# batra-mlp-lab/visdial

Hardware: AMD Instinct MI355X
Metric: QA-rounds/sec training mn-att-ques-im-hist+disc (batch 20x10x100) (higher is better)
Workload: dtype f32 operands and results; the option recurrence multiplies the EXACT 3-way bf16 split of both operands (9 bf16 MFMA products per fp32 product, f32 accumulate: fp32-grade, errors at the f32 MFMA's own level) -- its two step kernels and its weight-gradient contraction; f32 MFMA (v_mfma_f32_32x32x2_f32

## Files before the change

### visdial_amd/csrc/lstm.hip

```cpp
#include "gemm_core.h"
#include "split_core.h"

extern "C" int vd_gemm_tn_acc(const float* A, int64_t lda, const float* B, int64_t ldb, float* C, int64_t ldc, int M,
                              int N, int K, int flags, void* stream);

#define VD_LSTM_CELL(E, PI, PF, PO, PG, CP)   \
  gi.E = km * vd_sigmoid(PI);                 \
  gf.E = km * vd_sigmoid(PF);                 \
  go.E = km * vd_sigmoid(PO);                 \
  gg.E = km * vd_tanh(PG);                    \
  c.E = gf.E * (CP) + gi.E * gg.E;            \
  h.E = go.E * vd_tanh(c.E);
#define VD_XYZW(M) M(x) M(y) M(z) M(w)
#define VD_ADD4(a, b) a.x += b.x; a.y += b.y; a.z += b.z; a.w += b.w;

template <bool C16 = false>
struct EpiLstmFwdT {
  const float* xproj;
  long xld;
  const int* tok_gather;
  const int* tok_mask;
  const float* c_prev;
  float* gates;
  float* c_out;
// ... 322 lines not shown
  __device__ __forceinline__ long kstep() const { return 1; }
};

#define VD_LSTM_GRAD(E, G, CT, CP, DCV, LTR)                                                                   \
  {                                                                                                            \
    float gi_ = G[0].E, gf_ = G[1].E, go_ = G[2].E;                                                            \
    float pi_ = 0.f, pf_ = 0.f, po_ = 0.f;                              \
    if constexpr (!(LTR)) pi_ = gi_ * (1.f - gi_), pf_ = gf_ * (1.f - gf_), po_ = go_ * (1.f - go_);           \
    if constexpr (C16) {                \
      pi_ = gi_ < 0.f ? (1.f + gi_) * -gi_ : pi_;  gi_ = gi_ < 0.f ? 1.f + gi_ : gi_;                          \
      pf_ = gf_ < 0.f ? (1.f + gf_) * -gf_ : pf_;  gf_ = gf_ < 0.f ? 1.f + gf_ : gf_;                          \
      po_ = go_ < 0.f ? (1.f + go_) * -go_ : po_;  go_ = go_ < 0.f ? 1.f + go_ : go_;                          \
    }                                                                                                          \
    const float tc = vd_tanh(CT.E);                                                                            \
    const float d = DCV.E + dh.E * go_ * (1.f - tc * tc);                                                      \
    ai.E = LTR ? d * G[3].E * gi_ * (1.f - gi_) : d * G[3].E * pi_;                                            \
    af.E = LTR ? d * CP.E * gf_ * (1.f - gf_) : d * CP.E * pf_;                                                \
    ao.E = LTR ? dh.E * tc * go_ * (1.f - go_) : dh.E * tc * po_;                                              \
    ag.E = d * gi_ * (1.f - G[3].E * G[3].E);                                                                  \
    dn.E = d * gf_;                                                                                            \
  }

template <int NT, int BATCH = (NT == 1 ? 2 : 1), bool TWO = true, bool C16 = false>
struct EpiLstmBwd {
  const float* dh_a;
  const float* dh_b;
  float* gates;
  const float* c_t;
  const float* c_prev;
  float* dc;
  int dc_first;
  int H;
  vd_bf16_bits* da16 = nullptr;
  static constexpr bool HAS_DIST = NT == 1 && !C16;
  struct DOps {
    float4 g[4], ct, cp, dcv, dha, dhb;
  };
  __device__ __forceinline__ bool dist_ok() const { return true; }
  __device__ __forceinline__ void dist_load(DOps& q, int row0, int col0, int lane, int grp, int M) const {
    const int j = col0 + (lane & 7) * 4;
    const int row = row0 + grp * 8 + (lane >> 3);
    const int rc = row < M ? row : M - 1;
    const long o = (long)rc * H + j;
    const float* gr = gates + (long)rc * 4 * H + j;
    const float4 z = make_float4(0.f, 0.f, 0.f, 0.f);
    q.g[0] = *reinterpret_cast<const float4*>(gr);
    q.g[1] = *reinterpret_cast<const float4*>(gr + H);
    q.g[2] = *reinterpret_cast<const float4*>(gr + 2 * H);
    q.g[3] = *reinterpret_cast<const float4*>(gr + 3 * H);
    q.ct = *reinterpret_cast<const float4*>(c_t + o);
    q.cp = c_prev ? *reinterpret_cast<const float4*>(c_prev + o) : z;
    q.dcv = dc_first ? z : *reinterpret_cast<const float4*>(dc + o);
    q.dha = dh_a ? *reinterpret_cast<const float4*>(dh_a + o) : z;
    q.dhb = dh_b ? *reinterpret_cast<const float4*>(dh_b + o) : z;
  }
  __device__ __forceinline__ void dist_store(const float4 (&a)[1], const DOps& q, int row0, int col0, int lane, int grp, int M) const {
    const int j = col0 + (lane & 7) * 4;
    const int row = row0 + grp * 8 + (lane >> 3);
    if (row >= M || j >= H) return;
    float4 dh = a[0], ai, af, ao, ag, dn;
    dh.x += q.dha.x + q.dhb.x; dh.y += q.dha.y + q.dhb.y; dh.z += q.dha.z + q.dhb.z; dh.w += q.dha.w + q.dhb.w;
#define VD_GRAD(E) VD_LSTM_GRAD(E, q.g, q.ct, q.cp, q.dcv, true)
    VD_XYZW(VD_GRAD)
#undef VD_GRAD
    float* gr = gates + (long)row * 4 * H + j;
    *reinterpret_cast<float4*>(gr) = ai;
// ... 10 lines not shown
    }
  }
  struct Slot {
    float4 g[4], ct, cp, dcv, dhx;
    vd_u32x2 g16[4];
  };
  struct Rsrc {
    __amdgpu_buffer_rsrc_t g, ct, cp, dc, dh1, dh2, g16;
  };
  __device__ __forceinline__ void load_slot_buf(Slot& L, const Rsrc& R, unsigned o4, unsigned og4, unsigned uH4) const {
    if constexpr (C16) {
      L.g16[0] = __builtin_amdgcn_raw_buffer_load_b64(R.g, og4 >> 1, 0, 0);
      L.g16[1] = __builtin_amdgcn_raw_buffer_load_b64(R.g, og4 >> 1, uH4 >> 1, 0);
      L.g16[2] = __builtin_amdgcn_raw_buffer_load_b64(R.g, og4 >> 1, uH4, 0);
      L.g16[3] = __builtin_amdgcn_raw_buffer_load_b64(R.g, og4 >> 1, 3 * (uH4 >> 1), 0);
    } else {
    L.g[0] = vd_buf_ld4(R.g, og4, 0);
    L.g[1] = vd_buf_ld4(R.g, og4, uH4);
    L.g[2] = vd_buf_ld4(R.g, og4, 2 * uH4);
    L.g[3] = vd_buf_ld4(R.g, og4, 3 * uH4);
    }
    L.ct = vd_buf_ld4(R.ct, o4, 0);
    const float4 z = make_float4(0.f, 0.f, 0.f, 0.f);
    L.cp = c_prev ? vd_buf_ld4(R.cp, o4, 0) : z;
    L.dcv = dc_first ? z : vd_buf_ld4(R.dc, o4, 0);
    L.dhx = (dh_a || dh_b) ? vd_buf_ld4(R.dh1, o4, 0) : z;
  }
  __device__ __forceinline__ void operator()(const f32x16 (&acc)[NT], int row0, int col0, int lane, int M,
                                             int N, float* scr) const {
    const int rl = lane >> 3, cl = (lane & 7) * 4;
    const bool two_dh = TWO && dh_a && dh_b;
    const Rsrc R{vd_rsrc(gates), vd_rsrc(c_t), vd_rsrc(c_prev), vd_rsrc(dc), vd_rsrc(dh_a ? dh_a : dh_b), vd_rsrc(dh_b), vd_rsrc(da16)};
    const unsigned uH4 = (unsigned)H * 4u;
#pragma unroll
    for (int jt = 0; jt < NT; ++jt) {
      float4 d4[4];
      tile_to_rows(acc[jt], scr, lane, d4);
      if (jt == 0) VD_T(3);
      const int j = col0 + jt * 32 + cl;
      const int jc = j < N ? j : N - 4;
#pragma unroll
      for (int pp = 0; pp < 4; pp += BATCH) {
        Slot L[BATCH];
        unsigned o4[BATCH], og4[BATCH];
#pragma unroll
        for (int q = 0; q < BATCH; ++q) {
          const int row = row0 + (pp + q) * 8 + rl;
          o4[q] = (unsigned)(row < M ? row : M - 1) * uH4 + (unsigned)jc * 4u;
          og4[q] = 4u * o4[q] - 12u * (unsigned)jc;
          load_slot_buf(L[q], R, o4[q], og4[q], uH4);
        }
        __builtin_amdgcn_sched_barrier(0);
#pragma unroll
        for (int q = 0; q < BATCH; ++q) {
          Slot& C = L[q];
          if constexpr (C16) {
#pragma unroll
            for (int gk = 0; gk < 4; ++gk) C.g[gk] = vd_bf16x4_unpack(C.g16[gk]);
          }
          float4 dh = d4[pp + q];
          VD_ADD4(dh, C.dhx)
          const int row = row0 + (pp + q) * 8 + rl;
          if constexpr (TWO) {
            if (two_dh) {
              const float4 t = vd_buf_ld4(R.dh2, o4[q], 0);
              VD_ADD4(dh, t)
            }
          }
          float4 ai, af, ao, ag, dn;
#define VD_GRAD(E) VD_LSTM_GRAD(E, C.g, C.ct, C.cp, C.dcv, false)
          VD_XYZW(VD_GRAD)
#undef VD_GRAD
          if (row < M && j < N) {
            if constexpr (C16) {
              vd_buf_st4_bf16(R.g, og4[q] >> 1, 0, ai);
              vd_buf_st4_bf16(R.g, og4[q] >> 1, uH4 >> 1, af);
              vd_buf_st4_bf16(R.g, og4[q] >> 1, uH4, ao);
              vd_buf_st4_bf16(R.g, og4[q] >> 1, 3 * (uH4 >> 1), ag);
            } else {
            vd_buf_st4(R.g, og4[q], 0, ai);
            vd_buf_st4(R.g, og4[q], uH4, af);
            vd_buf_st4(R.g, og4[q], 2 * uH4, ao);
            vd_buf_st4(R.g, og4[q], 3 * uH4, ag);
            }
            vd_buf_st4(R.dc, o4[q], 0, dn);
            if (!C16 && da16) {
              vd_buf_st4_bf16(R.g16, og4[q] >> 1, 0, ai);
              vd_buf_st4_bf16(R.g16, og4[q] >> 1, uH4 >> 1, af);
              vd_buf_st4_bf16(R.g16, og4[q] >> 1, uH4, ao);
              vd_buf_st4_bf16(R.g16, og4[q] >> 1, 3 * (uH4 >> 1), ag);
            }
          }
        }
      }
    }
  }
};

using CfgF9 = GemmCfg<4, 1, 4, 16, 0, 4, 41984>;
using CfgB1 = GemmCfg<4, 1, 4, 32, 0, 3>;
using CfgB11 = GemmCfg<4, 1, 2, 16, 0, 4, 41984>;
using CfgFbf16 = GemmCfg<4, 1, 4, 32, 0, 3, 0, 1>;
using CfgBbf16 = GemmCfg<4, 1, 2, 32, 0, 3, 0, 1>;
#ifndef VD_C16_LDS
#define VD_C16_LDS 41984
#endif
using CfgF9bf16 = GemmCfg<4, 1, 4, 16, 0, 4, VD_C16_LDS, 1>;
using CfgB11bf16 = GemmCfg<4, 1, 2, 16, 0, 4, VD_C16_LDS, 1>;
using CfgFwdSmallA = GemmCfg<1, 4, 4, 8, 0, 3>;
using CfgFwdSmallC = GemmCfg<1, 4, 4, 8, 0, 4>;
using CfgBwdSmallD = GemmCfg<1, 4, 1, 32, 2, 4>;
using CfgTickFwdBf16 = GemmCfg<1, 4, 4, 16, 0, 3, 0, 1>;
using CfgTickBwdBf16 = GemmCfg<1, 4, 1, 32, 0, 4, 0, 1>;

__global__ void __launch_bounds__(256) wh_gate_transpose_kernel(const float* __restrict__ Wh,
                                                                float* __restrict__ WhT, int H, int plain = 0) {
  __shared__ float tile[32][33];
  const int vt = blockIdx.x, kt = blockIdx.y;
  const int jb = vt >> 2, g = vt & 3;
  const int tx = threadIdx.x & 31, ty = threadIdx.x >> 5;
  const long src_col = plain ? (long)vt * 32 : (long)g * H + jb * 32;
#pragma unroll
  for (int i = 0; i < 4; ++i) {
    const int k = kt * 32 + ty + i * 8;
    tile[ty + i * 8][tx] = Wh[(long)k * 4 * H + src_col + tx];
  }
// ... 61 lines not shown
  const int N = P.N, H = P.H;
  if (h_prev) {
    if constexpr (Epi::STEP_BF16) {
      if (P.bf16 && t > 0)
        return launch_gemm_glds<CfgF9bf16, false>(N, 4 * H, H / 2, 1, reinterpret_cast<const float*>(P.h16 + (long)(t - 1) * N * H), (long)H / 2,
                                                  reinterpret_cast<const float*>(P.w.W16), (long)H / 2, epi, s);
      if (P.bf16) return launch_gemm<CfgFbf16>(N, 4 * H, H, 1, SrcRow{h_prev, H}, SrcRow{P.w.WhT, H}, epi, s);
    }
    if constexpr (Epi::STEP_SPLIT) {
      if (P.split) return launch_gemm_split(P.split, N, 4 * H, H, h_prev, (long)H, P.w.W3, (long)H, 4L * H * H, epi, s);
    }
    if (P.glds) return launch_gemm_glds<CfgF9, false>(N, 4 * H, H, 1, h_prev, (long)H, P.w.WhT, (long)H, epi, s);
  }
  auto generic = [&](auto a) {
    SrcKGate4 b{P.Wh, 4L * H, H};
    if (N >= VD_THROUGHPUT_ROWS) return launch_gemm<CfgF9>(N, 4 * H, h_prev ? H : 0, 1, a, b, epi, s);
    return launch_gemm<CfgFwdSmallA>(N, 4 * H, h_prev ? H : 0, 1, a, b, epi, s);
  };
  if constexpr (EpiARowsOf<Epi>::value) {
    if (h_prev) return generic(SrcRowTree{h_prev, H, epi.tok_mask, epi.parent});
  }
  return generic(SrcRow{h_prev, H});
}

struct LstmBwdPlan {
  int N, H;
  const float* Wh;
  int split;
  LstmWeights w;
  vd_bf16_bits* da16;
};
template <class E>
static E lstm_bwd_epi(const EpiLstmBwd<2>& e) {
  return E{e.dh_a, e.dh_b, e.gates, e.c_t, e.c_prev, e.dc, e.dc_first, e.H, e.da16};
}

static int lstm_step_bwd(const LstmBwdPlan& P, const float* da_next, const vd_bf16_bits* da16_next, const EpiLstmBwd<2>& e, hipStream_t s) {
  const int N = P.N, H = P.H, K = da_next ? 4 * H : 0;
  const bool one_dh = !(e.dh_a && e.dh_b);
  SrcRow a{da_next, 4L * H};
  SrcRow b{P.Wh, 4L * H};
  if (P.split && K > 0 && one_dh)
    return launch_gemm_split(P.split, N, H, K, da_next, 4L * H, P.w.W3, 4L * H, 4L * H * H, lstm_bwd_epi<EpiLstmBwd<4, 2, false>>(e), s);
  if (N < VD_THROUGHPUT_ROWS)
    return launch_gemm<CfgBwdSmallD>(N, H, K, 1, a, b, lstm_bwd_epi<EpiLstmBwd<1>>(e), s);
  if (e.da16 && K > 0) {
    if (da16_next && P.w.W16 && K % 32 == 0)
      return launch_gemm_glds<CfgB11bf16, false>(N, H, K / 2, 1, reinterpret_cast<const float*>(da16_next), 2L * H,
                                                 reinterpret_cast<const float*>(P.w.W16), 2L * H, e, s);
    return launch_gemm<CfgBbf16>(N, H, K, 1, a, b, e, s);
  }
  if (!e.da16 && K > 0 && vd_lstm_glds_bwd_fits(N, H)) {
    if (one_dh) return launch_gemm_glds<CfgB11, false>(N, H, K, 1, da_next, 4L * H, P.Wh, 4L * H, lstm_bwd_epi<EpiLstmBwd<2, 2, false>>(e), s);
    return launch_gemm_glds<CfgB11, false>(N, H, K, 1, da_next, 4L * H, P.Wh, 4L * H, e, s);
  }
  return launch_gemm<CfgB11>(N, H, K, 1, a, b, e, s);
}

struct SrcKSel {
  static constexpr bool KMAJOR = true;
  static constexpr bool PLAIN = true;
  const float* p;
  long ld;
  int H;
  int gate4;
  __device__ __forceinline__ const float* ptr(int vc, int k) const {
    int col = vc;
// ... 189 lines not shown
  VD_CHECK_ARG(!live || tok_mask, "vd_lstm_forward: VD_FLAG_LIVE_PREFIX needs tok_mask");
  hipStream_t s = (hipStream_t)stream;
  const long NH = (long)N * H;
  LstmFwdPlan P{N, H, Wh};
  P.bf16 = (flags & VD_FLAG_BF16) && vd_lstm_bf16_fits(N, H);
  P.glds = !P.bf16 && !hold && T > 1 && vd_lstm_glds_fwd_fits(N, H);
  P.split = P.glds ? vd_split_nprod(flags) : 0;
  if (int rc0 = lstm_weights(Wh, H, P.glds || (P.bf16 && (T > 1 || h0)), P.split, P.bf16 && T > 1, s, &P.w)) return rc0;
  vd_bf16_bits* h16 = nullptr;
  if (P.bf16) {
    if (int rc0 = vd_bf16_shadow_get(0, h, (size_t)T * NH, &h16)) return rc0;
  } else {
    vd_bf16_shadow_invalidate(h, (size_t)(state_only ? 2 : T) * NH);
  }
  P.h16 = h16;
  if (gates) vd_bf16_shadow_invalidate(gates, (size_t)T * 4 * NH);
  for (int t = 0; t < T; ++t) {
    const long so = state_only ? (long)(t & 1) * NH : t * NH, sp = state_only ? (long)((t - 1) & 1) * NH : (t - 1) * NH;
    const float* hp = t ? h + sp : h0;
    const EpiLstmFwd e{xproj + (long)t * x_tstride, x_ld, tok_gather ? tok_gather + (long)t * N : nullptr,
                       tok_mask ? tok_mask + (long)t * N : nullptr,  t ? c + sp : c0, gates ? gates + (long)t * 4 * NH : nullptr,
                        c + so,  h + so, H, h16 ? h16 + t * NH : nullptr};
    int rc;
    if (tree) rc = lstm_step_fwd(P, t, hp, EpiLstmFwdTree{e, tok_mask + ((long)T + t) * N}, s);
    else if (hold) rc = lstm_step_fwd(P, t, hp, EpiLstmFwdHold{e, hp}, s);
    else if (state_only) rc = lstm_step_fwd(P, t, hp, EpiLstmFwdState{e}, s);
    else if (live) rc = lstm_step_fwd(P, t, hp, EpiLstmFwdLive{e}, s);
    else rc = lstm_step_fwd(P, t, hp, e, s);
    if (rc) return rc;
  }
  return VD_OK;
}

int vd_lstm_backward(const float* Wh, float* gates, const float* c, const float* c0, const float* dh_seq,
                     const float* dh_last, const float* dc_last, float* dc_work, float* dh0, const float* h_seq,
                     float* dWh_acc, int T, int N, int H, int flags, void* stream) {
  VD_CHECK_ARG(T >= 1 && N >= 0 && H > 0 && H % 32 == 0, "vd_lstm_backward: bad dims T=%d N=%d H=%d", T, N, H);
  VD_CHECK_ARG(Wh && gates && c && dc_work, "vd_lstm_backward: null pointer");
  VD_CHECK_ARG((h_seq == nullptr) == (dWh_acc == nullptr), "vd_lstm_backward: h_seq and dWh_acc go together");
  VD_CHECK_ARG((long)N * 4 * H * 4 < (1L << 32), "vd_lstm_backward: N=%d rows x 4H=%d exceed 4 GB per step: split the batch", N, 4 * H);
  hipStream_t s = (hipStream_t)stream;
  const long NH = (long)N * H;
  if (dc_last && dc_last != dc_work) VD_HIP(hipMemcpyAsync(dc_work, dc_last, NH * sizeof(float), hipMemcpyDeviceToDevice, s));
  const bool bf16 = (flags & VD_FLAG_BF16) && vd_lstm_bf16_fits(N, H);
  LstmBwdPlan P{N, H, Wh};
  P.split = !bf16 && T > 1 && vd_lstm_glds_bwd_fits(N, H) ? vd_split_nprod(flags) : 0;
  if (bf16) {
    if (int rc0 = vd_bf16_shadow_get(1, gates, (size_t)T * 4 * NH, &P.da16)) return rc0;
  } else {
    vd_bf16_shadow_invalidate(gates, (size_t)T * 4 * NH);
  }
  if (int rc0 = lstm_weights(Wh, H, false, P.split, bf16 && T > 1, s, &P.w)) return rc0;
  for (int t = T - 1; t >= 0; --t) {
    const bool last = (t == T - 1);
    float* g_t = gates + (long)t * 4 * NH;
    vd_bf16_bits* da16_t = P.da16 ? P.da16 + (long)t * 4 * NH : nullptr;
    const EpiLstmBwd<2> e{dh_seq ? dh_seq + t * NH : nullptr, (last && dh_last) ? dh_last : nullptr, g_t, c + t * NH, t ? c + (t - 1) * NH : c0,
                          dc_work, (last && !dc_last) ? 1 : 0, H, da16_t};
    const int rc = lstm_step_bwd(P, last ? nullptr : g_t + 4 * NH, (da16_t && !last) ? da16_t + 4 * NH : nullptr, e, s);
    if (rc) return rc;
  }
  int rc = VD_OK;
  if (dWh_acc && T > 1) {
    rc = vd_gemm_tn_acc(h_seq, H, gates + 4 * NH, 4L * H, dWh_acc, 4L * H, H, 4 * H, (T - 1) * N, flags & (VD_FLAG_BF16 | VD_FLAG_SPLIT9), s);
    if (rc) return rc;
  }
  if (dh0) {
    SrcRow a{gates, 4L * H};
    SrcRow b{Wh, 4L * H};
    EpiStore<4> e{dh0, H, nullptr, VD_ACT_NONE, 0};
    rc = launch_gemm<CfgB1>(N, H, 4 * H, 1, a, b, e, s);
    if (rc) return rc;
  }
  return VD_OK;
}

}

template <class Cfg>
static int lstm2_forward_ticks(const vd_lstm2_fwd_t* st, int nstacks, int H, int Tmax, hipStream_t stream) {
  for (int tau = 0; tau < Tmax + 2; ++tau) {
    GroupArgs<TickFwdProb, 3 * VD_MAX_STACKS> g;
    g.nprob = 0;
    for (int s = 0; s < nstacks; ++s) {
      const vd_lstm2_fwd_t& S = st[s];
      const long NH = (long)S.N * H;
      for (int layer = 1; layer <= 2; ++layer) {
        const int t = layer == 1 ? tau : tau - 2;
        if (t < 0 || t >= S.T) continue;
        float* gates = layer == 1 ? S.gates1 : S.gates2;
        float* h = layer == 1 ? S.h1 : S.h2;
        float* c = layer == 1 ? S.c1 : S.c2;
        const int rows = S.nact ? S.nact[t] : S.N;
        if (rows <= 0) continue;
        TickFwdProb& P = g.p[g.nprob++];
        P.M = rows; P.N = 4 * H; P.K = t ? H : 0;
        P.a = SrcRow{t ? h + (t - 1) * NH : h, H};
        P.b = SrcKSel{layer == 1 ? S.Wh1 : S.Wh2, 4L * H, H, 1};
        P.e.kind = 0;
        P.e.f.xproj = gates + (long)t * 4 * NH; P.e.f.xld = 4L * H;
        P.e.f.tok_gather = nullptr;
        P.e.f.tok_mask = S.tok_mask ? S.tok_mask + (long)t * S.N : nullptr;
        P.e.f.c_prev = t ? c + (t - 1) * NH : nullptr;
        P.e.f.gates = gates + (long)t * 4 * NH; P.e.f.c_out = c + t * NH; P.e.f.h_out = h + t * NH; P.e.f.H = H;
        P.e.s = EpiStore<4>{nullptr, 0, nullptr, 0, 0};
      }
      const int t = tau - 1;
// ... 103 lines not shown
```

### visdial_amd/csrc/paths.h

```cpp
#pragma once
#include "common.h"

static inline int vd_precision_flags(int lstmBf16) {
  switch (lstmBf16) {
    case 0: return 0;
    case 1: return VD_FLAG_BF16;
    case 3: return VD_FLAG_SPLIT3;
    case 6: return VD_FLAG_SPLIT6;
    case 9: return VD_FLAG_SPLIT9;
    default: return -1;
  }
}
static inline int vd_split_nprod(int flags) {
  return (flags & VD_FLAG_SPLIT9) ? 9 : (flags & VD_FLAG_SPLIT6) ? 6 : (flags & VD_FLAG_SPLIT3) ? 3 : 0;
}

constexpr long VD_THROUGHPUT_ROWS = 2048;
constexpr int VD_LSTM_FWD_TILE_BIG = 128, VD_LSTM_FWD_TILE_SMALL = 32;
static inline int vd_lstm_fwd_row_tile(long N) { return N >= VD_THROUGHPUT_ROWS ? VD_LSTM_FWD_TILE_BIG : VD_LSTM_FWD_TILE_SMALL; }
static inline bool vd_lstm_glds_fwd_fits(long N, int H) { return N >= VD_THROUGHPUT_ROWS && H % 32 == 0 && N * H * 4 < (1L << 32); }
static inline bool vd_lstm_glds_bwd_fits(long N, int H) { return N >= VD_THROUGHPUT_ROWS && H % 32 == 0 && N * 4 * H * 4 < (1L << 32); }
static inline bool vd_lstm_bf16_fits(long N, int H) { return N >= VD_THROUGHPUT_ROWS && H % 32 == 0; }
static inline bool vd_lstm_c16_fits(long N, int H) { return N >= VD_THROUGHPUT_ROWS && H % 128 == 0; }

static inline bool vd_tn_kmajor_fits(long M, long N, long K) { return M % 128 == 0 && N % 128 == 0 && K >= 1024; }
constexpr int VD_SPLIT_TN_BM = 256, VD_SPLIT_TN_BN = 128;
static inline bool vd_tn_split_tiles(long M, long N) { return M % VD_SPLIT_TN_BM == 0 && N % VD_SPLIT_TN_BN == 0; }

static inline bool vd_img_split_ok(long rows, int H, int Kc) {
  return rows >= 128 && H % 16 == 0 && Kc % 16 == 0 && rows * (H > Kc ? H : Kc) * 4 < (1L << 32);
}

static inline bool vd_lhood_fused_fits(long rows, long ldh, long V, long ldw, int H) {
  return H >= 64 && H % 16 == 0 && V >= 128 && ldh % 4 == 0 && ldw % 4 == 0 && rows * ldh * 4 < (1L << 32) && V * ldw * 4 < (1L << 32);
}
static inline bool vd_lhood_prefix_fits(int T, long rows) { return T >= 1 && T < 256 && rows >= 1; }
```

### visdial_amd/csrc/rt_core.h

```cpp
#pragma once
#include <math.h>
#include <stdarg.h>
#include <stdlib.h>
#include <string.h>

#include <algorithm>
#include <map>
#include <memory>
#include <numeric>
#include <random>
#include <string>
#include <vector>

#include "../../include/visdial_hip.h"
#include "common.h"
#include "paths.h"
#include "rt_switches.h"

static_assert(VD_OK == 0 && VD_ERR_ARG == -1, "rt_switches.h returns the two as literals: it includes no common.h");

int vd_lstm2_forward_p(const vd_lstm2_fwd_t* st, int nstacks, int H, int flags, hipStream_t stream);
int vd_lstm2_backward_p(const vd_lstm2_bwd_t* st, int nstacks, int H, int flags, hipStream_t stream);

int vd_img_drop_gather(const float* pre, const uint8_t* mask1, float* xdrop, int N, int R, int S2, int H, float scale, hipStream_t stream);
int vd_img_common_forward_p(const float* pre, const uint8_t* mask1, const float* xdrop, const float* Wc, const float* bc, const float* qc,
                            const uint8_t* mask2, float* iqc, int N, int R, int S2, int H, int Kc, float scale, int flags, hipStream_t stream);
int vd_img_tr_backward_p(const float* dz, const float* Wc, const float* p, const float* datt, const uint8_t* mask1, float* dpre, int N, int R,
                         int S2, int H, int Kc, float scale, int flags, hipStream_t stream);
int vd_img_common_wgrad_p(const float* dz, const float* pre, const uint8_t* mask1, const float* xdrop, float* dWc, int N, int R, int S2, int H,
                          int Kc, float scale, int flags, hipStream_t stream);

int vd_mn_attention_round_p(const float* Q, int64_t q_ld, const float* Hm, float* P, float* hAtt, float* Qout, int B, int R, int r, int H,
                            hipStream_t stream);
int vd_hrea_attention_round_p(const float* sq, const float* sh, const float* Hm, float* P, float* att, int B, int R, int r, int H,
                              hipStream_t stream);
int vd_round_embed_p(const float* emb, const int32_t* tok, int T, int N, int R, int r, int32_t* tok_r, float* x, int E, hipStream_t stream);
int vd_rows_cat_p(float* dst, int64_t dst_ld, const float* const* src, const int64_t* ld, const int* cols, int nparts, int64_t rows,
                  hipStream_t stream);

int vd_gemm_nn_live_p(const float* A, int64_t lda, const float* B, int64_t ldb, const float* bias, float* C, int64_t ldc, int M, int N, int K,
                      const int32_t* tok_mask, int row_tile, hipStream_t stream);
int vd_lhood_order_p(const int32_t* tok_in, const int32_t* target, int T, int64_t rows, int C, int32_t* perm, int32_t* rep, int32_t* tok_in_s,
                     int32_t* target_s, int32_t* work, int32_t* info, hipStream_t stream);
int64_t vd_lhood_order_work_ints(int T, int64_t rows);
int vd_lhood_sum_p(const float* nll, const int32_t* act, int64_t n_act, int T, int64_t rows, int C, const int32_t* perm, float* out, int64_t ldo,
                   hipStream_t stream);

int vd_lhood_lse_p(const float* h, int64_t ldh, int64_t rows, const int32_t* act, int64_t n_act, const float* W, int64_t ldw, const float* bias,
                   int V, int H, float* lse, hipStream_t stream);
int vd_lhood_edge_sum_p(const float* h, int64_t ldh, const int32_t* node_row, const float* lse, const int32_t* enode, const int32_t* etgt, int T,
                        int64_t rows, int C, const float* W, int64_t ldw, const float* bias, int H, float* out, int64_t ldo, hipStream_t stream);

int vd_sample_draw_trunc_p(const float* logits, int64_t ld, int64_t rows, int V, int32_t* tok, const double* uniforms, double temperature,
                           int top_k, double top_p, int step, int beam_len, int end_token, int32_t* hist, double* loglik, int32_t* status,
                           hipStream_t stream);
// ... 32 lines not shown
};

struct SeqTok {
  int T = 0, N = 0;
  bool present = false, sorted = false;
  int32_t* tok = nullptr;
  std::vector<int32_t> nact;
  int32_t *tok_sorted = nullptr, *fwd_idx = nullptr, *inv_idx = nullptr, *perm = nullptr, *inv = nullptr, *nact_dev = nullptr;
  int32_t *act = nullptr, *act1 = nullptr, *prev1 = nullptr;
  int n_act = 0, n_act1 = 0;
};

struct TreeChunk {
  int o0 = 0, C = 0, Tl = 0, Nw = 0;
  long n_nodes = 0;
  std::vector<int32_t> widths;
  int32_t* mask2 = nullptr;
  int32_t* node_row = nullptr;
  int32_t *enode = nullptr, *etgt = nullptr;
};

struct BatchSlot {
  int B = 0;
  bool tree_ok = false;
  std::vector<TreeChunk> tree;
  SeqTok q, h, opt, ain, aout, oin, oout;
  float* img = nullptr;
  int32_t* gt = nullptr;
  std::vector<int32_t> gt_host;
  bool has_gt = false;
  int32_t* opt_uid = nullptr;
  int opt_total = 0;
  int32_t *opt_sort_off = nullptr, *opt_sort_perm = nullptr;
  bool cached = false;
  uint64_t cache_stamp = 0;
  std::vector<int32_t> miss_keys, opt_host;
  hipEvent_t ready = nullptr;
  hipEvent_t done = nullptr;
  bool used = false;
  bool uploaded = false;
  std::map<std::string, DevBuf> bufs, pinned;
};

struct RowIndex {
  int T = 0;
  std::vector<int32_t> keys;
  std::vector<int32_t> table;
  int32_t size() const { return T ? (int32_t)(keys.size() / (size_t)T) : 0; }
  void reset(int T_) {
    T = T_;
    keys.clear();
    table.assign(1024, -1);
  }
  size_t home(const int32_t* row) const {
    uint64_t h = 1469598103934665603ull;
    for (int t = 0; t < T; ++t) h = (h ^ (uint32_t)row[t]) * 1099511628211ull;
    return (size_t)(h ^ (h >> 29)) & (table.size() - 1);
  }
  int32_t find(const int32_t* row) const {
    for (size_t pos = home(row);; pos = (pos + 1) & (table.size() - 1)) {
      const int32_t u = table[pos];
      if (u < 0) return -1;
      if (memcmp(keys.data() + (size_t)u * T, row, (size_t)T * sizeof(int32_t)) == 0) return u;
    }
  }
  int32_t add(const int32_t* row) {
// ... 449 lines not shown
```

### visdial_amd/csrc/rt_decoders.h

```cpp
#pragma once
#include "rt_encoders.h"

namespace vdrt {

int option_cache_resolve(vd_model* m, BatchSlot& sl, const int32_t* options, long NO, int To, hipStream_t s);

struct Decoder {
  virtual ~Decoder() {}
  virtual void declare(vd_model* m) = 0;
  virtual int forward_backward(vd_model* m, BatchSlot& b, bool only_forward) = 0;
  virtual int retrieve(vd_model* m, BatchSlot& b) = 0;
  virtual int retrieve_lhood(vd_model*, BatchSlot&) {
    vd_set_error("vd_model_retrieve_lhood: the live-row log-likelihood head scores candidates of decoder 'gen'; this model's decoder is 'disc'");
    return VD_ERR_ARG;
  }
  virtual int gen_begin(vd_model*, const int32_t*, int) { return no_gen(); }
  virtual int gen_step(vd_model*, const int32_t*, float*) { return no_gen(); }
  virtual int gen_select(vd_model*, const int32_t*, int) { return no_gen(); }
  virtual int gen_beam_search(vd_model*, int, int, int, int, int32_t*, double*) { return no_gen(); }
  virtual int gen_sample(vd_model*, int, int, int, double, const double*, int32_t*, double*) { return no_gen(); }
  static int no_gen() {
    vd_set_error("sampling / beam search only for the generative decoder (model.lua:436-438)");
    return VD_ERR_STATE;
  }
// ... 129 lines not shown
    VD_TRY(vd_score_ce(optH, enc_out, b.gt, scores, loss_rows, dedup ? d_optH_full : d_optH, d_enc, N, O, (int)H, 1.0f / N, s));
    if (dedup && !only_forward) {
      VD_TRY(vd_memset(d_optH, 0, (long)NO * H * 4, s));
      VD_TRY(vd_embed_scatter_acc(d_optH, b.opt_uid, nullptr, d_optH_full, NOfull, (int)H, 1.f, s));
    }
    VD_TRY(stage_loss(m, loss_rows, N, false, s));
    m->scores = scores;
    m->prof_valid = !only_forward;
    if (only_forward) return VD_OK;
    VD_TRY(fork_stream(m, s, sd));
    float *dc, *dtab;
    int32_t* perm = b.opt_sort_perm;
    VD_TRY(ws_get(m, "opt.dc", (size_t)NO * H, &dc));
    VD_TRY(ws_get(m, "opt.dtable", (size_t)(V + 1) * 4 * H, &dtab));
    VD_CHECK_ARG(perm, "decoder 'disc': the batch slot carries no option-token sort");
    VD_TRY(vd_memset(dtab, 0, (V + 1) * 4 * H * 4, sd));
    VD_HIP(hipEventRecord(m->ev_prof[2], s));
    m->wg_active = m->streams && m->s_wg && (flags & VD_FLAG_BF16) != 0;
    m->wg_used = false;
    auto enc_bwd = [&]() -> int {
      VdRange r("encoder backward");
      VD_TRY(m->enc->backward(m, sd, b, d_enc));
      VD_PROBE_REC(1, sd);
      if (m->wg_used) VD_PROBE_REC(2, m->s_wg);
      if (m->wg_used) {
        VD_TRY(fork_stream(m, sd, m->s_wg));
        VD_HIP(hipEventRecord(m->ev_enc_grads, m->s_wg));
      } else {
        VD_HIP(hipEventRecord(m->ev_enc_grads, sd));
      }
      m->enc_grads_recorded = true;
      return VD_OK;
    };
    {
      VdRange r("disc: option LSTM backward");
      if (c16) VD_TRY(vd_lstm_backward_c16(Wopt + E * 4 * H, gates16, c, d_optH, dc, To, NO, (int)H, s));
      else VD_TRY(vd_lstm_backward(Wopt + E * 4 * H, gates, c, nullptr, nullptr, d_optH, nullptr, dc, nullptr, nullptr, nullptr, To, NO, (int)H, flags, s));
    }
    VD_HIP(hipEventRecord(m->ev_prof[3], s));
    VD_TRY(enc_bwd());
    VdRange rwg("disc: table gradient + dWh");
    VD_TRY(fork_stream(m, s, sd));
    if (c16) VD_TRY(vd_segment_rowsum_acc_bf16(gates16, 4 * H, b.opt.tok, perm, (long)To * NO, (int)(4 * H), dtab, 4 * H, sd));
    else VD_TRY(vd_segment_rowsum_acc(gates, 4 * H, b.opt.tok, perm, (long)To * NO, (int)(4 * H), dtab, 4 * H, sd));
    VD_TRY(vd_colsum_acc(dtab, 4 * H, (int)V + 1, (int)(4 * H), Gp(m, "opt.b"), sd));
    VD_TRY(vd_gemm_tn_acc(Wp(m, "embed"), E, dtab, 4 * H, Gp(m, "opt.W"), 4 * H, (int)E, (int)(4 * H), (int)V + 1, 0, sd));
    VD_HIP(hipEventRecord(m->ev_prof[4], s));
    if (To > 1 && c16)
      VD_TRY(vd_gemm_tn_acc_bf16(h16, gates16 + (long)NO * 4 * H, Gp(m, "opt.W") + E * 4 * H, 4 * H, (int)H, (int)(4 * H), (To - 1) * NO, s));
    else if (To > 1)
      VD_TRY(vd_gemm_tn_acc(h, H, gates + (long)NO * 4 * H, 4 * H, Gp(m, "opt.W") + E * 4 * H, 4 * H, (int)H, (int)(4 * H), (To - 1) * NO,
                            flags & (VD_FLAG_BF16 | VD_FLAG_SPLIT9), s));
    VD_HIP(hipEventRecord(m->ev_prof[5], s));
    VD_TRY(vd_gemm_nt(dtab, 4 * H, Wopt, 4 * H, nullptr, Gp(m, "embed"), E, (int)V + 1, (int)E, (int)(4 * H), VD_ACT_NONE, 2, sd));
    VD_PROBE_REC(3, sd);
    VD_TRY(join_stream(m, sd, s));
    if (m->wg_used) VD_TRY(join_stream(m, m->s_wg, s));
    m->wg_active = m->wg_used = false;
    VD_PROBE_REC(4, s);
    return VD_OK;
  }
  int retrieve(vd_model* m, BatchSlot& b) override {
    if (m->sw.retrieve_rollout && m->use_hist) return retrieve_rollout(m, b);
    return forward_backward(m, b, true);
  }

  int retrieve_rollout(vd_model* m, BatchSlot& b) {
    VD_TRY(refuse_round_rollout_in_training(m, "vd_model_retrieve"));
    if (m->training) {
      vd_set_error("vd_model_retrieve: this model was created with VD_RETRIEVE_ROLLOUT = 1, and a rollout re-runs the encoder once per round: "
                   "under training-mode dropout the passes would not describe one model; call vd_model_set_training(0) first");
      return VD_ERR_STATE;
    }
    VD_CHECK_ARG(b.opt.present && !b.cached, "decoder 'disc' needs batch.options");
    const int N = b.q.N, O = m->p.numOptions, NOfull = N * O, NO = b.opt.N, R = m->p.maxQuesCount, B = N / R;
    const bool dedup = b.opt_uid != nullptr;
    VD_CHECK_ARG(dedup ? NO <= NOfull : NO == NOfull, "decoder 'disc': %d option rows for %d x %d candidates", NO, N, O);
// ... 687 lines not shown
```

### visdial_amd/csrc/runtime.hip

```cpp
#include "rt_decoders.h"

using namespace vdrt;

vd_model::~vd_model() {}

namespace {

int upload_tokens(BatchSlot& sl, SeqTok& ss, const std::string& tag, const int32_t* rows_major, int N, int T, bool sorted, hipStream_t s,
                  int rollout_R = 0) {
  ss.T = T;
  ss.N = N;
  ss.present = true;
  ss.sorted = sorted;
  const size_t TN = (size_t)T * N;
  const size_t total = sorted ? 7 * TN + 2 * (size_t)N + T : TN;
  int32_t* stage = nullptr;
  VD_TRY(pin_get(sl.pinned, tag + ".stage", total * sizeof(int32_t), (void**)&stage));
  int32_t* tok = stage;
  std::vector<int> len(sorted ? N : 0);
  for (int n = 0; n < N; ++n) {
    int first = T;
    for (int t = 0; t < T; ++t) {
      const int32_t v = rows_major[(size_t)n * T + t];
      tok[(size_t)t * N + n] = v;
// ... 457 lines not shown
  const bool disc = m->dec_name == "disc";
  VD_CHECK_ARG(!disc || (hb->options && hb->To > 0), "vd_model_upload_batch: decoder 'disc' needs options");
  VdRange r("vd_model_upload_batch");
  BatchSlot& sl = m->slot[m->cur < 0 ? 0 : (m->cur ^ 1)];
  hipStream_t s = m->s_side;
  if (sl.used) VD_HIP(hipStreamWaitEvent(s, sl.done, 0));
  if (sl.uploaded) VD_HIP(hipEventSynchronize(sl.ready));
  sl.uploaded = true;
  sl.B = hb->B;
  const int R = m->p.maxQuesCount, N = hb->B * R, O = m->p.numOptions;
  const long NO = (long)N * O;
  for (SeqTok* t : {&sl.q, &sl.h, &sl.opt, &sl.ain, &sl.aout, &sl.oin, &sl.oout}) t->present = false;
  VD_TRY(upload_tokens(sl, sl.q, "q", hb->ques_fwd, N, hb->Tq, m->is_graph, s));
  const bool hist_wave = !m->is_graph && m->p.numLayers == 2;
  const bool rollout = m->sw.beam_rollout || m->sw.retrieve_rollout;
  VD_CHECK_ARG(!(rollout && m->use_hist) || hb->Th >= hb->Tq,
               "vd_model_upload_batch: %s = 1 needs a history width Th = %d >= the question width Tq = %d",
               m->sw.beam_rollout ? "VD_BEAM_ROLLOUT" : "VD_RETRIEVE_ROLLOUT", hb->Th, hb->Tq);
  if (m->use_hist) VD_TRY(upload_tokens(sl, sl.h, "h", hb->hist, N, hb->Th, m->is_graph || hist_wave, s, rollout ? R : 0));
  if (m->use_im) {
    const size_t img_n = (size_t)hb->B * (m->is_att ? (size_t)m->p.imgSpatialSize * m->p.imgSpatialSize : 1) * m->p.imgFeatureSize;
    float* ip = nullptr;
    VD_TRY(pin_get(sl.pinned, "img.stage", img_n * sizeof(float), (void**)&ip));
    memcpy(ip, hb->img_feat, img_n * sizeof(float));
    VD_TRY(dev_get(sl.bufs, "img", img_n * sizeof(float), (void**)&sl.img));
    VD_HIP(hipMemcpyAsync(sl.img, ip, img_n * sizeof(float), hipMemcpyHostToDevice, s));
  }
  if (disc) {
    sl.opt_uid = nullptr;
    sl.opt_total = (int)NO;
    sl.cached = false;
    const int To = hb->To;
    bool dedup = false;
    if (m->ocache.capacity > 0 && !m->training) {
      sl.opt_host.assign(hb->options, hb->options + (size_t)NO * To);
      VD_TRY(option_cache_resolve(m, sl, sl.opt_host.data(), NO, To, s));
    } else if (NO > 1) {
      std::vector<int32_t> uid((size_t)NO), uniq;
      uniq.reserve((size_t)NO * To);
      const size_t cap = (size_t)1 << (64 - __builtin_clzll((unsigned long long)(2 * NO)));
      std::vector<int32_t> table(cap, -1);
      int U = 0;
      for (long r = 0; r < NO; ++r) {
        const int32_t* row = hb->options + (size_t)r * To;
        uint64_t h = 1469598103934665603ull;
        for (int t = 0; t < To; ++t) h = (h ^ (uint32_t)row[t]) * 1099511628211ull;
        size_t pos = (size_t)(h ^ (h >> 29)) & (cap - 1);
        for (;;) {
          const int32_t u = table[pos];
          if (u < 0) {
            table[pos] = U;
            uid[r] = U++;
            uniq.insert(uniq.end(), row, row + To);
            break;
          }
          if (memcmp(uniq.data() + (size_t)u * To, row, (size_t)To * sizeof(int32_t)) == 0) {
            uid[r] = u;
            break;
          }
          pos = (pos + 1) & (cap - 1);
        }
      }
      if ((double)U <= 0.95 * (double)NO) {
        dedup = true;
        VD_TRY(upload_tokens(sl, sl.opt, "opt", uniq.data(), U, To, false, s));
        int32_t* up = nullptr;
        VD_TRY(pin_get(sl.pinned, "opt.uid.stage", (size_t)NO * sizeof(int32_t), (void**)&up));
        memcpy(up, uid.data(), (size_t)NO * sizeof(int32_t));
        VD_TRY(dev_get(sl.bufs, "opt.uid", (size_t)NO * sizeof(int32_t), (void**)&sl.opt_uid));
        VD_HIP(hipMemcpyAsync(sl.opt_uid, up, (size_t)NO * sizeof(int32_t), hipMemcpyHostToDevice, s));
      }
    }
    if (!dedup && !sl.cached) VD_TRY(upload_tokens(sl, sl.opt, "opt", hb->options, (int)NO, hb->To, false, s));
    sl.opt_sort_off = sl.opt_sort_perm = nullptr;
    if (!sl.cached) {
      const long V1 = (long)m->p.vocabSize + 1, n = (long)sl.opt.T * sl.opt.N;
      int32_t* work;
      VD_TRY(dev_get(sl.bufs, "opt.sort_off", (size_t)(V1 + 1) * sizeof(int32_t), (void**)&sl.opt_sort_off));
      VD_TRY(dev_get(sl.bufs, "opt.sort_work", (size_t)2 * V1 * sizeof(int32_t), (void**)&work));
      VD_TRY(dev_get(sl.bufs, "opt.sort_perm", (size_t)n * sizeof(int32_t), (void**)&sl.opt_sort_perm));
      VD_TRY(vd_token_sort(sl.opt.tok, n, (int)V1, sl.opt_sort_off, work, sl.opt_sort_perm, s));
    }
  }
  if (!disc && hb->answer_in && hb->answer_out) {
    VD_TRY(upload_tokens(sl, sl.ain, "ain", hb->answer_in, N, hb->Ta, false, s));
    VD_TRY(upload_tokens(sl, sl.aout, "aout", hb->answer_out, N, hb->Ta, false, s));
  }
  sl.tree_ok = false;
  if (!disc && hb->option_in && hb->option_out) {
    VD_TRY(upload_tokens(sl, sl.oin, "oin", hb->option_in, (int)NO, hb->To, false, s));
    VD_TRY(upload_tokens(sl, sl.oout, "oout", hb->option_out, (int)NO, hb->To, false, s));
    if (m->sw.lhood_tree) VD_TRY(build_lhood_tree(m, sl, hb->option_in, hb->option_out, N, O, hb->To, s));
  }
  sl.has_gt = hb->answer_ind != nullptr;
  sl.gt_host.assign(N, 0);
  int32_t* gp = nullptr;
  VD_TRY(pin_get(sl.pinned, "gt.stage", (size_t)N * sizeof(int32_t), (void**)&gp));
  for (int n = 0; n < N; ++n) {
    const int g = hb->answer_ind ? hb->answer_ind[n] - 1 : 0;
    VD_CHECK_ARG(!hb->answer_ind || (g >= 0 && g < O), "vd_model_upload_batch: answer_ind[%d] = %d out of 1..%d", n, g + 1, O);
    sl.gt_host[n] = g;
    gp[n] = g;
  }
  VD_TRY(dev_get(sl.bufs, "gt", (size_t)N * sizeof(int32_t), (void**)&sl.gt));
  VD_HIP(hipMemcpyAsync(sl.gt, gp, (size_t)N * sizeof(int32_t), hipMemcpyHostToDevice, s));
  VD_HIP(hipEventRecord(sl.ready, s));
  m->uploaded = (int)(&sl - m->slot);
  m->lhood_exec = -1;
  return VD_OK;
}

static int begin_step(vd_model* m, bool zero_grads, BatchSlot** out) {
  VD_CHECK_ARG(m && m->uploaded >= 0, "no batch uploaded");
  m->cur = m->uploaded;
// ... 177 lines not shown
```

Before: 8862.

## Fuse pad-token gate-gradient sum into option LSTM backward epilogue

Inside the LSTM backward step epilogue, rows whose token is the pad token (0) have their gate gradients reduced through LDS and atomically added into a small per-column pad_sum buffer. The segment row-sum for the embedding table then skips the sorted pad rows (the perm is offset by the host-counted pad count), and pad_sum is added into the pad row of dtab with an axpby. This targets the usually large, serial pad segment in the table-gradient reduction. In exchange the epilogue gains token loads, a ballot, LDS traffic and global atomics on every step, and the host counts pad tokens for each batch.

After: 8930, median of 6. No clear change (+0.8%).

```diff
diff --git a/visdial_amd/csrc/lstm.hip b/visdial_amd/csrc/lstm.hip
--- a/visdial_amd/csrc/lstm.hip
+++ b/visdial_amd/csrc/lstm.hip
@@ -378,6 +378,8 @@
   int dc_first;
   int H;
   vd_bf16_bits* da16 = nullptr;
+  const int* tok = nullptr;
+  float* pad_sum = nullptr;
   static constexpr bool HAS_DIST = NT == 1 && !C16;
   struct DOps {
     float4 g[4], ct, cp, dcv, dha, dhb;
@@ -454,6 +456,19 @@
     const bool two_dh = TWO && dh_a && dh_b;
     const Rsrc R{vd_rsrc(gates), vd_rsrc(c_t), vd_rsrc(c_prev), vd_rsrc(dc), vd_rsrc(dh_a ? dh_a : dh_b), vd_rsrc(dh_b), vd_rsrc(da16)};
     const unsigned uH4 = (unsigned)H * 4u;
+    const bool psum = !C16 && !(NT == 2 && BATCH == 2) && tok && pad_sum;
+    unsigned padm = 0;
+    if (psum) {
+      int tk[4];
+#pragma unroll
+      for (int p = 0; p < 4; ++p) {
+        const int row = row0 + p * 8 + rl;
+        tk[p] = tok[row < M ? row : M - 1];
+      }
+#pragma unroll
+      for (int p = 0; p < 4; ++p) padm |= (row0 + p * 8 + rl < M && tk[p] == 0) ? 1u << p : 0u;
+    }
+    const bool wsum = psum && __ballot(padm != 0) != 0;
 #pragma unroll
     for (int jt = 0; jt < NT; ++jt) {
       float4 d4[4];
@@ -461,10 +476,26 @@
       if (jt == 0) VD_T(3);
       const int j = col0 + jt * 32 + cl;
       const int jc = j < N ? j : N - 4;
+      float psv[2] = {0.f, 0.f};
 #pragma unroll
       for (int pp = 0; pp < 4; pp += BATCH) {
         Slot L[BATCH];
         unsigned o4[BATCH], og4[BATCH];
+        float4 si = make_float4(0.f, 0.f, 0.f, 0.f), sf = si, so = si, sg = si;
+        auto ps_flush = [&]() {
+          asm volatile("" ::: "memory");
+          float* w = scr + rl * 128 + cl;
+          *reinterpret_cast<float4*>(w) = si;
+          *reinterpret_cast<float4*>(w + 32) = sf;
+          *reinterpret_cast<float4*>(w + 64) = so;
+          *reinterpret_cast<float4*>(w + 96) = sg;
+          asm volatile("" ::: "memory");
+#pragma unroll
+          for (int k = 0; k < 2; ++k)
+#pragma unroll
+            for (int r = 0; r < 8; ++r) psv[k] += scr[r * 128 + k * 64 + lane];
+          asm volatile("" ::: "memory");
+        };
 #pragma unroll
         for (int q = 0; q < BATCH; ++q) {
           const int row = row0 + (pp + q) * 8 + rl;
@@ -493,6 +524,12 @@
 #define VD_GRAD(E) VD_LSTM_GRAD(E, C.g, C.ct, C.cp, C.dcv, false)
           VD_XYZW(VD_GRAD)
 #undef VD_GRAD
+          if (wsum) {
+            const bool pz = (padm >> (pp + q)) & 1u;
+#define VD_PSUM(E) si.E += pz ? ai.E : 0.f; sf.E += pz ? af.E : 0.f; so.E += pz ? ao.E : 0.f; sg.E += pz ? ag.E : 0.f;
+            VD_XYZW(VD_PSUM)
+#undef VD_PSUM
+          }
           if (row < M && j < N) {
             if constexpr (C16) {
               vd_buf_st4_bf16(R.g, og4[q] >> 1, 0, ai);
@@ -514,6 +551,14 @@
             }
           }
         }
+        if (wsum) ps_flush();
+      }
+      if (wsum) {
+#pragma unroll
+        for (int k = 0; k < 2; ++k) {
+          const int cc = k * 64 + lane, ju = col0 + jt * 32 + (cc & 31);
+          if (ju < N) unsafeAtomicAdd(pad_sum + (long)(cc >> 5) * H + ju, psv[k]);
+        }
       }
     }
   }
@@ -641,7 +686,7 @@
 };
 template <class E>
 static E lstm_bwd_epi(const EpiLstmBwd<2>& e) {
-  return E{e.dh_a, e.dh_b, e.gates, e.c_t, e.c_prev, e.dc, e.dc_first, e.H, e.da16};
+  return E{e.dh_a, e.dh_b, e.gates, e.c_t, e.c_prev, e.dc, e.dc_first, e.H, e.da16, e.tok, e.pad_sum};
 }
 
 static int lstm_step_bwd(const LstmBwdPlan& P, const float* da_next, const vd_bf16_bits* da16_next, const EpiLstmBwd<2>& e, hipStream_t s) {
@@ -897,14 +942,18 @@
   return VD_OK;
 }
 
-int vd_lstm_backward(const float* Wh, float* gates, const float* c, const float* c0, const float* dh_seq,
-                     const float* dh_last, const float* dc_last, float* dc_work, float* dh0, const float* h_seq,
-                     float* dWh_acc, int T, int N, int H, int flags, void* stream) {
+}
+
+int vd_lstm_backward_p(const float* Wh, float* gates, const float* c, const float* c0, const float* dh_seq,
+                       const float* dh_last, const float* dc_last, float* dc_work, float* dh0, const float* h_seq,
+                       float* dWh_acc, int T, int N, int H, int flags, const int32_t* tok, float* pad_sum, hipStream_t s) {
   VD_CHECK_ARG(T >= 1 && N >= 0 && H > 0 && H % 32 == 0, "vd_lstm_backward: bad dims T=%d N=%d H=%d", T, N, H);
+  VD_CHECK_ARG((tok == nullptr) == (pad_sum == nullptr), "vd_lstm_backward: tok and pad_sum go together");
+  VD_CHECK_ARG(!pad_sum || vd_lstm_pad_sum_fits(N, flags),
+               "vd_lstm_backward: the pad-row sum exists in the throughput step kernels of a split pass only (N=%d flags=%d)", N, flags);
   VD_CHECK_ARG(Wh && gates && c && dc_work, "vd_lstm_backward: null pointer");
   VD_CHECK_ARG((h_seq == nullptr) == (dWh_acc == nullptr), "vd_lstm_backward: h_seq and dWh_acc go together");
   VD_CHECK_ARG((long)N * 4 * H * 4 < (1L << 32), "vd_lstm_backward: N=%d rows x 4H=%d exceed 4 GB per step: split the batch", N, 4 * H);
-  hipStream_t s = (hipStream_t)stream;
   const long NH = (long)N * H;
   if (dc_last && dc_last != dc_work) VD_HIP(hipMemcpyAsync(dc_work, dc_last, NH * sizeof(float), hipMemcpyDeviceToDevice, s));
   const bool bf16 = (flags & VD_FLAG_BF16) && vd_lstm_bf16_fits(N, H);
@@ -921,7 +970,7 @@
     float* g_t = gates + (long)t * 4 * NH;
     vd_bf16_bits* da16_t = P.da16 ? P.da16 + (long)t * 4 * NH : nullptr;
     const EpiLstmBwd<2> e{dh_seq ? dh_seq + t * NH : nullptr, (last && dh_last) ? dh_last : nullptr, g_t, c + t * NH, t ? c + (t - 1) * NH : c0,
-                          dc_work, (last && !dc_last) ? 1 : 0, H, da16_t};
+                          dc_work, (last && !dc_last) ? 1 : 0, H, da16_t, tok ? tok + (long)t * N : nullptr, pad_sum};
     const int rc = lstm_step_bwd(P, last ? nullptr : g_t + 4 * NH, (da16_t && !last) ? da16_t + 4 * NH : nullptr, e, s);
     if (rc) return rc;
   }
@@ -938,6 +987,15 @@
     if (rc) return rc;
   }
   return VD_OK;
+}
+
+extern "C" {
+
+int vd_lstm_backward(const float* Wh, float* gates, const float* c, const float* c0, const float* dh_seq,
+                     const float* dh_last, const float* dc_last, float* dc_work, float* dh0, const float* h_seq,
+                     float* dWh_acc, int T, int N, int H, int flags, void* stream) {
+  return vd_lstm_backward_p(Wh, gates, c, c0, dh_seq, dh_last, dc_last, dc_work, dh0, h_seq, dWh_acc, T, N, H, flags, nullptr, nullptr,
+                            (hipStream_t)stream);
 }
 
 }
diff --git a/visdial_amd/csrc/paths.h b/visdial_amd/csrc/paths.h
--- a/visdial_amd/csrc/paths.h
+++ b/visdial_amd/csrc/paths.h
@@ -22,6 +22,9 @@
 static inline bool vd_lstm_glds_bwd_fits(long N, int H) { return N >= VD_THROUGHPUT_ROWS && H % 32 == 0 && N * 4 * H * 4 < (1L << 32); }
 static inline bool vd_lstm_bf16_fits(long N, int H) { return N >= VD_THROUGHPUT_ROWS && H % 32 == 0; }
 static inline bool vd_lstm_c16_fits(long N, int H) { return N >= VD_THROUGHPUT_ROWS && H % 128 == 0; }
+static inline bool vd_lstm_pad_sum_fits(long N, int flags) {
+  return N >= VD_THROUGHPUT_ROWS && !(flags & VD_FLAG_BF16) && vd_split_nprod(flags) != 0;
+}
 
 static inline bool vd_tn_kmajor_fits(long M, long N, long K) { return M % 128 == 0 && N % 128 == 0 && K >= 1024; }
 constexpr int VD_SPLIT_TN_BM = 256, VD_SPLIT_TN_BN = 128;
diff --git a/visdial_amd/csrc/rt_core.h b/visdial_amd/csrc/rt_core.h
--- a/visdial_amd/csrc/rt_core.h
+++ b/visdial_amd/csrc/rt_core.h
@@ -21,6 +21,10 @@
 
 int vd_lstm2_forward_p(const vd_lstm2_fwd_t* st, int nstacks, int H, int flags, hipStream_t stream);
 int vd_lstm2_backward_p(const vd_lstm2_bwd_t* st, int nstacks, int H, int flags, hipStream_t stream);
+
+int vd_lstm_backward_p(const float* Wh, float* gates, const float* c, const float* c0, const float* dh_seq, const float* dh_last,
+                       const float* dc_last, float* dc_work, float* dh0, const float* h_seq, float* dWh_acc, int T, int N, int H, int flags,
+                       const int32_t* tok, float* pad_sum, hipStream_t stream);
 
 int vd_img_drop_gather(const float* pre, const uint8_t* mask1, float* xdrop, int N, int R, int S2, int H, float scale, hipStream_t stream);
 int vd_img_common_forward_p(const float* pre, const uint8_t* mask1, const float* xdrop, const float* Wc, const float* bc, const float* qc,
@@ -119,6 +123,7 @@
   int32_t* opt_uid = nullptr;
   int opt_total = 0;
   int32_t *opt_sort_off = nullptr, *opt_sort_perm = nullptr;
+  long opt_n_pad = 0;
   bool cached = false;
   uint64_t cache_stamp = 0;
   std::vector<int32_t> miss_keys, opt_host;
diff --git a/visdial_amd/csrc/rt_decoders.h b/visdial_amd/csrc/rt_decoders.h
--- a/visdial_amd/csrc/rt_decoders.h
+++ b/visdial_amd/csrc/rt_decoders.h
@@ -185,17 +185,27 @@
       m->enc_grads_recorded = true;
       return VD_OK;
     };
+    float* pad_sum = nullptr;
+    const long n_pad = !c16 && vd_lstm_pad_sum_fits(NO, flags) ? b.opt_n_pad : 0;
+    if (n_pad > 0) {
+      VD_TRY(ws_get(m, "opt.pad_sum", (size_t)(4 * H), &pad_sum));
+      VD_TRY(vd_memset(pad_sum, 0, 4 * H * 4, s));
+    }
     {
       VdRange r("disc: option LSTM backward");
       if (c16) VD_TRY(vd_lstm_backward_c16(Wopt + E * 4 * H, gates16, c, d_optH, dc, To, NO, (int)H, s));
-      else VD_TRY(vd_lstm_backward(Wopt + E * 4 * H, gates, c, nullptr, nullptr, d_optH, nullptr, dc, nullptr, nullptr, nullptr, To, NO, (int)H, flags, s));
+      else VD_TRY(vd_lstm_backward_p(Wopt + E * 4 * H, gates, c, nullptr, nullptr, d_optH, nullptr, dc, nullptr, nullptr, nullptr, To, NO, (int)H, flags,
+                                     pad_sum ? b.opt.tok : nullptr, pad_sum, s));
     }
     VD_HIP(hipEventRecord(m->ev_prof[3], s));
     VD_TRY(enc_bwd());
     VdRange rwg("disc: table gradient + dWh");
     VD_TRY(fork_stream(m, s, sd));
     if (c16) VD_TRY(vd_segment_rowsum_acc_bf16(gates16, 4 * H, b.opt.tok, perm, (long)To * NO, (int)(4 * H), dtab, 4 * H, sd));
-    else VD_TRY(vd_segment_rowsum_acc(gates, 4 * H, b.opt.tok, perm, (long)To * NO, (int)(4 * H), dtab, 4 * H, sd));
+    else {
+      VD_TRY(vd_segment_rowsum_acc(gates, 4 * H, b.opt.tok, perm + n_pad, (long)To * NO - n_pad, (int)(4 * H), dtab, 4 * H, sd));
+      if (pad_sum) VD_TRY(vd_axpby(pad_sum, dtab, dtab, 4 * H, 1.f, 1.f, sd));
+    }
     VD_TRY(vd_colsum_acc(dtab, 4 * H, (int)V + 1, (int)(4 * H), Gp(m, "opt.b"), sd));
     VD_TRY(vd_gemm_tn_acc(Wp(m, "embed"), E, dtab, 4 * H, Gp(m, "opt.W"), 4 * H, (int)E, (int)(4 * H), (int)V + 1, 0, sd));
     VD_HIP(hipEventRecord(m->ev_prof[4], s));
diff --git a/visdial_amd/csrc/runtime.hip b/visdial_amd/csrc/runtime.hip
--- a/visdial_amd/csrc/runtime.hip
+++ b/visdial_amd/csrc/runtime.hip
@@ -513,6 +513,8 @@
     sl.cached = false;
     const int To = hb->To;
     bool dedup = false;
+    long n_pad_up = 0;
+    auto count_pad = [](const int32_t* t, size_t n) { return (long)std::count(t, t + n, 0); };
     if (m->ocache.capacity > 0 && !m->training) {
       sl.opt_host.assign(hb->options, hb->options + (size_t)NO * To);
       VD_TRY(option_cache_resolve(m, sl, sl.opt_host.data(), NO, To, s));
@@ -545,6 +547,7 @@
       if ((double)U <= 0.95 * (double)NO) {
         dedup = true;
         VD_TRY(upload_tokens(sl, sl.opt, "opt", uniq.data(), U, To, false, s));
+        n_pad_up = count_pad(uniq.data(), (size_t)U * To);
         int32_t* up = nullptr;
         VD_TRY(pin_get(sl.pinned, "opt.uid.stage", (size_t)NO * sizeof(int32_t), (void**)&up));
         memcpy(up, uid.data(), (size_t)NO * sizeof(int32_t));
@@ -552,8 +555,12 @@
         VD_HIP(hipMemcpyAsync(sl.opt_uid, up, (size_t)NO * sizeof(int32_t), hipMemcpyHostToDevice, s));
       }
     }
-    if (!dedup && !sl.cached) VD_TRY(upload_tokens(sl, sl.opt, "opt", hb->options, (int)NO, hb->To, false, s));
+    if (!dedup && !sl.cached) {
+      VD_TRY(upload_tokens(sl, sl.opt, "opt", hb->options, (int)NO, hb->To, false, s));
+      n_pad_up = count_pad(hb->options, (size_t)NO * To);
+    }
     sl.opt_sort_off = sl.opt_sort_perm = nullptr;
+    sl.opt_n_pad = 0;
     if (!sl.cached) {
       const long V1 = (long)m->p.vocabSize + 1, n = (long)sl.opt.T * sl.opt.N;
       int32_t* work;
@@ -561,6 +568,7 @@
       VD_TRY(dev_get(sl.bufs, "opt.sort_work", (size_t)2 * V1 * sizeof(int32_t), (void**)&work));
       VD_TRY(dev_get(sl.bufs, "opt.sort_perm", (size_t)n * sizeof(int32_t), (void**)&sl.opt_sort_perm));
       VD_TRY(vd_token_sort(sl.opt.tok, n, (int)V1, sl.opt_sort_off, work, sl.opt_sort_perm, s));
+      sl.opt_n_pad = n_pad_up;
     }
   }
   if (!disc && hb->answer_in && hb->answer_out) {
```
